# david-macmahon/BLDistributedDataProducts.jl

Hardware: AMD Instinct MI355X
Metric: filterbank GB/s reduced (node) + % HBM roofline, 8-bank 0000 band (higher is better)
Workload: dtype f32

## Files before the change

### bldistributeddataproducts.jl_amd/csrc/bslz4.hip

```cpp
#include <algorithm>
#include <cstring>
#include <vector>

#include "bldp_impl.h"

namespace {

inline uint32_t be32(const uint8_t *p) {
  return (uint32_t)p[0] << 24 | (uint32_t)p[1] << 16 | (uint32_t)p[2] << 8 | p[3];
}
inline uint64_t be64(const uint8_t *p) { return (uint64_t)be32(p) << 32 | be32(p + 4); }

__host__ __device__ inline uint64_t transpose8(uint64_t x) {
  uint64_t t;
  t = (x ^ (x >> 7)) & 0x00AA00AA00AA00AAull;
  x = x ^ t ^ (t << 7);
  t = (x ^ (x >> 14)) & 0x0000CCCC0000CCCCull;
  x = x ^ t ^ (t << 14);
  t = (x ^ (x >> 28)) & 0x00000000F0F0F0F0ull;
  x = x ^ t ^ (t << 28);
  return x;
}

int64_t lz4_block_host(const uint8_t *src, size_t slen, uint8_t *dst, size_t dcap) {
  size_t ip = 0, op = 0;
  while (ip < slen) {
    const uint8_t token = src[ip++];
    size_t lit = token >> 4;
    if (lit == 15) {
      uint8_t b;
      do {
        if (ip >= slen) return -1;
        b = src[ip++];
        lit += b;
      } while (b == 255);
    }
    if (ip + lit > slen || op + lit > dcap) return -1;
    memcpy(dst + op, src + ip, lit);
    ip += lit;
    op += lit;
    if (ip >= slen) break;
    if (ip + 2 > slen) return -1;
    const size_t off = (size_t)src[ip] | (size_t)src[ip + 1] << 8;
    ip += 2;
    size_t ml = token & 15;
    if (ml == 15) {
      uint8_t b;
      do {
        if (ip >= slen) return -1;
        b = src[ip++];
        ml += b;
      } while (b == 255);
    }
    ml += 4;
    if (off == 0 || off > op || op + ml > dcap) return -1;
    for (size_t i = 0; i < ml; ++i) dst[op + i] = dst[op - off + i];
    op += ml;
  }
  return (int64_t)op;
}

void bitunshuffle_host(const uint8_t *planes, uint8_t *out, size_t n, size_t es) {
  const size_t rowb = n / 8;
  for (size_t g = 0; g < rowb; ++g)
    for (size_t j = 0; j < es; ++j) {
      uint64_t x = 0;
      for (int k = 0; k < 8; ++k) x |= (uint64_t)planes[(j * 8 + k) * rowb + g] << (8 * k);
      x = transpose8(x);
      for (int t = 0; t < 8; ++t) out[(8 * g + t) * es + j] = (uint8_t)(x >> (8 * t));
    }
}

struct Task {
  uint64_t src;
  uint64_t dst;
  uint32_t clen;
  uint32_t nelem;
};
constexpr uint32_t RAW = 0xFFFFFFFFu;

struct ChunkDesc {
  uint64_t src, len, dst;
  uint64_t n, block;
  uint32_t nfull, last, tail;
  uint32_t task0;
};

int describe_chunk(const uint8_t *c, uint64_t len, uint64_t src, uint64_t dst, int es,
                   ChunkDesc *d) {
  if (len < 12) return bldp::set_error(BLDP_EINVAL, "bslz4: chunk shorter than its header");
  const uint64_t nb = be64(c);
  const uint32_t bb = be32(c + 8);
  if (nb % es || bb % es || bb == 0 || (bb / es) % 8 || bb > (1u << 24))
    return bldp::set_error(BLDP_EINVAL, "bslz4: bad header (bytes %llu, block %u, elem %d)",
                           (unsigned long long)nb, bb, es);
  d->src = src;
  d->len = len;
  d->dst = dst;
  d->n = nb / es;
  d->block = bb / es;
  d->nfull = (uint32_t)(d->n / d->block);
  uint64_t last = d->n % d->block;
  d->last = (uint32_t)(last - last % 8);
  d->tail = (uint32_t)(d->n - (uint64_t)d->nfull * d->block - d->last);
  return BLDP_OK;
}

inline uint32_t ntasks(const ChunkDesc &d) {
  return d.nfull + (d.last ? 1 : 0) + (d.tail ? 1 : 0);
}

__host__ __device__ inline uint32_t lz4_bound(uint32_t n) { return n + n / 255 + 16; }

__device__ inline uint32_t be32_dev(const uint8_t *p) {
  return (uint32_t)p[0] << 24 | (uint32_t)p[1] << 16 | (uint32_t)p[2] << 8 | p[3];
}

__global__ __launch_bounds__(64) void k_bslz4_plan(const uint8_t *__restrict__ comp,
                                                   const ChunkDesc *__restrict__ chunks,
                                                   int nchunk, int es, uint32_t cap,
                                                   Task *__restrict__ tasks, int *err) {
  const int k = blockIdx.x * 64 + threadIdx.x;
  if (k >= nchunk) return;
  const ChunkDesc d = chunks[k];
  uint64_t pos = d.src + 12, e = 0;
  const uint64_t end = d.src + d.len;
  const uint32_t nblk = d.nfull + (d.last ? 1 : 0);
  for (uint32_t b = 0; b < nblk; ++b) {
    const uint32_t ne = b < d.nfull ? (uint32_t)d.block : d.last;
    if (pos + 4 > end) { atomicOr(err, 2); return; }
    const uint32_t cl = be32_dev(comp + pos);
    if (cl > cap || pos + 4 + cl > end) { atomicOr(err, 2); return; }
    tasks[d.task0 + b] = Task{pos + 4, d.dst + e * es, cl, ne};
    pos += 4 + cl;
    e += ne;
  }
  if (pos + (uint64_t)d.tail * es != end) { atomicOr(err, 4); return; }
  if (d.tail) tasks[d.task0 + nblk] = Task{pos, d.dst + e * es, RAW, d.tail};
}

int plan_chunk(const uint8_t *c, uint64_t len, uint64_t src0, uint64_t dst0, int es,
               std::vector<Task> &tasks, uint64_t *out_bytes, uint32_t *max_block) {
  if (len < 12) return bldp::set_error(BLDP_EINVAL, "bslz4: chunk shorter than its header");
  const uint64_t nb = be64(c);
  const uint32_t bb = be32(c + 8);
  if (nb % es || bb % es || bb == 0 || (bb / es) % 8)
    return bldp::set_error(BLDP_EINVAL, "bslz4: bad header (bytes %llu, block %u, elem %d)",
                           (unsigned long long)nb, bb, es);
  const uint64_t n = nb / es, block = bb / es;
  uint64_t pos = 12, e = 0;
  const uint64_t nfull = n / block;
  uint64_t last = n % block;
  last -= last % 8;
  for (uint64_t k = 0; k < nfull + (last ? 1 : 0); ++k) {
    const uint64_t ne = k < nfull ? block : last;
    if (pos + 4 > len) return bldp::set_error(BLDP_EINVAL, "bslz4: truncated block header");
    const uint32_t cl = be32(c + pos);
    if (cl == RAW || pos + 4 + cl > len)
      return bldp::set_error(BLDP_EINVAL, "bslz4: block %llu overruns the chunk",
                             (unsigned long long)k);
    tasks.push_back(Task{src0 + pos + 4, dst0 + e * es, cl, (uint32_t)ne});
    *max_block = std::max<uint32_t>(*max_block, std::max<uint32_t>(cl, (uint32_t)(ne * es)));
    pos += 4 + cl;
    e += ne;
  }
  const uint64_t tail = n - e;
  if (pos + tail * es != len)
    return bldp::set_error(BLDP_EINVAL, "bslz4: %llu trailing bytes, expected %llu",
                           (unsigned long long)(len - pos), (unsigned long long)(tail * es));
  if (tail) tasks.push_back(Task{src0 + pos, dst0 + e * es, RAW, (uint32_t)tail});
  *out_bytes = nb;
  return BLDP_OK;
}

__global__ __launch_bounds__(64) void k_bslz4(const uint8_t *__restrict__ comp,
                                              const Task *__restrict__ tasks, int ntask,
                                              uint8_t *__restrict__ out, int es, uint32_t cap,
                                              int *err) {
  extern __shared__ uint8_t lds[];
  const int lane = threadIdx.x;
  if (*err & 6) return;
  const Task t = tasks[blockIdx.x];
  if (t.clen == RAW) {
    for (uint32_t i = lane; i < t.nelem * (uint32_t)es; i += 64) out[t.dst + i] = comp[t.src + i];
    return;
  }
  uint8_t *in = lds, *dec = lds + cap;
  const uint32_t clen = t.clen, nbytes = t.nelem * (uint32_t)es;
  if (clen > cap) {
    if (lane == 0) atomicOr(err, 1);
    return;
  }
  for (uint32_t i = lane; i < clen; i += 64) in[i] = comp[t.src + i];
  __syncthreads();
  uint32_t ip = 0, op = 0;
  bool bad = false;
  while (ip < clen) {
    const uint32_t token = in[ip++];
    uint32_t lit = token >> 4;
    if (lit == 15) {
      uint32_t b;
      do {
        if (ip >= clen) { bad = true; break; }
        b = in[ip++];
        lit += b;
      } while (b == 255);
      if (bad) break;
    }
    if (ip + lit > clen || op + lit > nbytes) { bad = true; break; }
    for (uint32_t i = lane; i < lit; i += 64) dec[op + i] = in[ip + i];
    ip += lit;
    op += lit;
    if (ip >= clen) break;
    if (ip + 2 > clen) { bad = true; break; }
    const uint32_t off = (uint32_t)in[ip] | (uint32_t)in[ip + 1] << 8;
    ip += 2;
    uint32_t ml = token & 15;
    if (ml == 15) {
      uint32_t b;
      do {
        if (ip >= clen) { bad = true; break; }
        b = in[ip++];
        ml += b;
      } while (b == 255);
      if (bad) break;
    }
    ml += 4;
    if (off == 0 || off > op || op + ml > nbytes) { bad = true; break; }
    __syncthreads();
    const uint32_t step = off < 64 ? off : 64;
    for (uint32_t r = 0; r < ml; r += step) {
      const uint32_t i = r + lane;
      if (lane < step && i < ml) dec[op + i] = dec[op - off + i];
      __syncthreads();
    }
    op += ml;
  }
  if (bad || op != nbytes) {
    if (lane == 0) atomicOr(err, 1);
    return;
  }
  __syncthreads();
  const uint32_t rowb = t.nelem / 8;
  if (es == 4) {
    for (uint32_t g = lane; g < rowb; g += 64) {
      uint32_t w[8] = {0, 0, 0, 0, 0, 0, 0, 0};
#pragma unroll
      for (int j = 0; j < 4; ++j) {
        uint64_t x = 0;
#pragma unroll
        for (int k = 0; k < 8; ++k) x |= (uint64_t)dec[(j * 8 + k) * rowb + g] << (8 * k);
        x = transpose8(x);
#pragma unroll
        for (int q = 0; q < 8; ++q) w[q] |= (uint32_t)((x >> (8 * q)) & 0xFF) << (8 * j);
      }
      uint32_t *o = reinterpret_cast<uint32_t *>(out + t.dst) + 8 * g;
#pragma unroll
      for (int q = 0; q < 8; ++q) o[q] = w[q];
    }
  } else {
    for (uint32_t g = lane; g < rowb; g += 64)
      for (int j = 0; j < es; ++j) {
        uint64_t x = 0;
        for (int k = 0; k < 8; ++k) x |= (uint64_t)dec[(j * 8 + k) * rowb + g] << (8 * k);
        x = transpose8(x);
        for (int q = 0; q < 8; ++q) out[t.dst + (8 * g + q) * es + j] = (uint8_t)(x >> (8 * q));
      }
  }
}

}

extern "C" {

BLDP_API int bldp_bslz4_info(const void *chunk, size_t nbytes, uint64_t *uncompressed_bytes,
                             uint32_t *block_bytes) {
  if (!chunk || nbytes < 12 || !uncompressed_bytes || !block_bytes)
    return bldp::set_error(BLDP_EINVAL, "bslz4: null pointer or short chunk");
  *uncompressed_bytes = be64((const uint8_t *)chunk);
  *block_bytes = be32((const uint8_t *)chunk + 8);
  return BLDP_OK;
}

BLDP_API int bldp_bslz4_decode_host(const void *chunk, size_t nbytes, int elem_size, void *out,
                                    size_t out_bytes) {
  if (!chunk || (!out && out_bytes) || elem_size <= 0)
    return bldp::set_error(BLDP_EINVAL, "bslz4: bad argument");
  std::vector<Task> tasks;
  uint64_t total = 0;
  uint32_t maxb = 0;
  int rc = plan_chunk((const uint8_t *)chunk, nbytes, 0, 0, elem_size, tasks, &total, &maxb);
  if (rc) return rc;
  if (total != out_bytes)
    return bldp::set_error(BLDP_EINVAL, "bslz4: chunk holds %llu bytes, output has %zu",
                           (unsigned long long)total, out_bytes);
  const uint8_t *c = (const uint8_t *)chunk;
  uint8_t *o = (uint8_t *)out;
  std::vector<uint8_t> dec(maxb);
  for (const Task &t : tasks) {
    const size_t nb = (size_t)t.nelem * elem_size;
    if (t.clen == RAW) {
      memcpy(o + t.dst, c + t.src, nb);
      continue;
    }
    if (lz4_block_host(c + t.src, t.clen, dec.data(), nb) != (int64_t)nb)
      return bldp::set_error(BLDP_EINVAL, "bslz4: corrupt LZ4 block at byte %llu",
                             (unsigned long long)t.src);
    bitunshuffle_host(dec.data(), o + t.dst, t.nelem, elem_size);
  }
  return BLDP_OK;
}

static int decode_launch(int nchunk, const uint8_t *comp_host, const uint8_t *comp_dev,
                         const uint64_t *chunk_off, const uint64_t *chunk_len, int elem_size,
                         uint8_t *out_dev, const uint64_t *out_off, const uint64_t *out_len,
                         int *derr_user, hipStream_t s, int **derr_used,
                         bldp::ScratchLease &lease, uint64_t host_base = 0) {
  if (nchunk < 0 || (nchunk && (!comp_host || !comp_dev || !chunk_off || !chunk_len ||
                                !out_dev || !out_off || !out_len)) ||
      elem_size <= 0 || elem_size > 64)
    return bldp::set_error(BLDP_EINVAL, "bslz4: bad argument");
  if (elem_size == 4 && ((uintptr_t)out_dev & 3))
    return bldp::set_error(BLDP_EINVAL, "bslz4: output must be 4-byte aligned");
  std::vector<ChunkDesc> descs(nchunk);
  uint64_t ntask = 0;
  uint32_t maxbb = 0;
  for (int k = 0; k < nchunk; ++k) {
    if (chunk_off[k] < host_base)
      return bldp::set_error(BLDP_EINVAL, "bslz4: chunk %d below the host staging base", k);
    int rc = describe_chunk(comp_host + (chunk_off[k] - host_base), chunk_len[k], chunk_off[k],
                            out_off[k],
                            elem_size, &descs[k]);
    if (rc) return rc;
    if (descs[k].n * (uint64_t)elem_size != out_len[k])
      return bldp::set_error(BLDP_EINVAL,
                             "bslz4: chunk %d decodes to %llu bytes, its output slot holds %llu",
                             k, (unsigned long long)(descs[k].n * elem_size),
                             (unsigned long long)out_len[k]);
    if (elem_size == 4 && (out_off[k] & 3))
      return bldp::set_error(BLDP_EINVAL, "bslz4: output offsets must be 4-byte aligned");
    descs[k].task0 = (uint32_t)ntask;
    ntask += ntasks(descs[k]);
    if (ntask > INT32_MAX) return bldp::set_error(BLDP_EINVAL, "bslz4: too many blocks");
    maxbb = std::max<uint32_t>(maxbb, (uint32_t)(descs[k].block * elem_size));
  }
  *derr_used = nullptr;
  if (ntask == 0) return BLDP_OK;
  const uint32_t cap = (lz4_bound(maxbb) + 15) & ~15u;
  if ((size_t)cap + (((size_t)maxbb + 15) & ~(size_t)15) > 64 * 1024)
    return bldp::set_error(BLDP_EINVAL, "bslz4: block of %u bytes exceeds the LDS plan", maxbb);
  const size_t dbytes = ((descs.size() * sizeof(ChunkDesc)) + 255) & ~(size_t)255;
  const size_t tbytes = ((ntask * sizeof(Task)) + 255) & ~(size_t)255;
  int rc = bldp::scratch_lease(s, dbytes + tbytes + 256, &lease);
  if (rc) return rc;
  void *ws = lease.ptr;
  ChunkDesc *ddesc = (ChunkDesc *)ws;
  Task *dtask = (Task *)((char *)ws + dbytes);
  int *derr = derr_user ? derr_user : (int *)((char *)ws + dbytes + tbytes);
  if (hipMemcpyAsync(ddesc, descs.data(), descs.size() * sizeof(ChunkDesc),
                     hipMemcpyHostToDevice, s) != hipSuccess ||
      (!derr_user && hipMemsetAsync(derr, 0, sizeof(int), s) != hipSuccess))
    return bldp::set_error(BLDP_EHIP, "bslz4: descriptor upload failed");
  hipLaunchKernelGGL(k_bslz4_plan, dim3((unsigned)((nchunk + 63) / 64)), dim3(64), 0, s,
                     comp_dev, ddesc, nchunk, elem_size, cap, dtask, derr);
  const uint32_t dcap = (maxbb + 15) & ~15u;
  hipLaunchKernelGGL(k_bslz4, dim3((unsigned)ntask), dim3(64), cap + dcap, s, comp_dev, dtask,
                     (int)ntask, out_dev, elem_size, cap, derr);
  hipError_t e = hipGetLastError();
  if (e != hipSuccess) return bldp::set_error(BLDP_EHIP, "bslz4 launch: %s", hipGetErrorString(e));
  *derr_used = derr;
  return BLDP_OK;
}

static int decode_error(int herr) {
  if (herr & 6) return bldp::set_error(BLDP_EINVAL, "bslz4: block table overruns a chunk");
  if (herr) return bldp::set_error(BLDP_EINVAL, "bslz4: corrupt LZ4 block on the device");
  return BLDP_OK;
}

BLDP_API int bldp_bslz4_decode_dev(int nchunk, const uint8_t *comp_host, const uint8_t *comp_dev,
                                   const uint64_t *chunk_off, const uint64_t *chunk_len,
                                   int elem_size, uint8_t *out_dev, const uint64_t *out_off,
                                   const uint64_t *out_len, void *stream) {
  hipStream_t s = (hipStream_t)stream;
  int *derr = nullptr;
  bldp::ScratchLease lease;
  int rc = decode_launch(nchunk, comp_host, comp_dev, chunk_off, chunk_len, elem_size, out_dev,
                         out_off, out_len, nullptr, s, &derr, lease);
  if (rc || !derr) return rc;
  int herr = 0;
  if (hipMemcpyAsync(&herr, derr, sizeof(int), hipMemcpyDeviceToHost, s) != hipSuccess ||
      hipStreamSynchronize(s) != hipSuccess)
    return bldp::set_error(BLDP_EHIP, "bslz4: synchronize failed");
  return decode_error(herr);
}

BLDP_API int bldp_bslz4_decode_dev_async(int nchunk, const uint8_t *comp_host,
                                         const uint8_t *comp_dev, const uint64_t *chunk_off,
                                         const uint64_t *chunk_len, int elem_size,
                                         uint8_t *out_dev, const uint64_t *out_off,
                                         const uint64_t *out_len, int *err_dev, void *stream) {
  if (!err_dev) return bldp::set_error(BLDP_EINVAL, "bslz4: null error word");
  int *derr = nullptr;
  bldp::ScratchLease lease;
  return decode_launch(nchunk, comp_host, comp_dev, chunk_off, chunk_len, elem_size, out_dev,
                       out_off, out_len, err_dev, (hipStream_t)stream, &derr, lease);
}

BLDP_API int bldp_bslz4_error(const int *err_dev, void *stream) {
  if (!err_dev) return bldp::set_error(BLDP_EINVAL, "bslz4: null error word");
  int herr = 0;
  hipStream_t s = (hipStream_t)stream;
  if (hipMemcpyAsync(&herr, err_dev, sizeof(int), hipMemcpyDeviceToHost, s) != hipSuccess ||
      hipStreamSynchronize(s) != hipSuccess)
    return bldp::set_error(BLDP_EHIP, "bslz4: synchronize failed");
  return decode_error(herr);
}

}

int bldp::bslz4_decode_async_at(int nchunk, const uint8_t *comp_host, uint64_t host_base,
                                const uint8_t *comp_dev, const uint64_t *chunk_off,
                                const uint64_t *chunk_len, int elem_size, uint8_t *out_dev,
                                const uint64_t *out_off, const uint64_t *out_len, int *err_dev,
                                hipStream_t s) {
  if (!err_dev) return bldp::set_error(BLDP_EINVAL, "bslz4: null error word");
  int *derr = nullptr;
  bldp::ScratchLease lease;
  return decode_launch(nchunk, comp_host, comp_dev, chunk_off, chunk_len, elem_size, out_dev,
                       out_off, out_len, err_dev, s, &derr, lease, host_base);
}
```

Before: 7394.

## Vectorize bslz4 staging, literal copies, match copies and bitshuffle output

Reworks the per-block LZ4 decode kernel in four places. Compressed input is staged into LDS with aligned 16-byte loads, literals are copied 8 bytes at a time, and match copies use a modular residue per lane so there is no per-step barrier. The es=4 bitshuffle transpose now reads dwords from LDS and writes 16-byte stores. These target byte-granular memory traffic and barrier stalls, at the cost of more registers (a 32-word array) and an extra 16 bytes of LDS per block.

```diff
diff --git a/bldistributeddataproducts.jl_amd/csrc/bslz4.hip b/bldistributeddataproducts.jl_amd/csrc/bslz4.hip
--- a/bldistributeddataproducts.jl_amd/csrc/bslz4.hip
+++ b/bldistributeddataproducts.jl_amd/csrc/bslz4.hip
@@ -3,6 +3,7 @@
 #include <vector>
 
 #include "bldp_impl.h"
+#include "bslz4_lanes.h"
 
 namespace {
 
@@ -173,25 +174,60 @@
   return BLDP_OK;
 }
 
+#ifndef BLDP_BSLZ4_STEPS
+#define BLDP_BSLZ4_STEPS 15
+#endif
+constexpr int kBslz4Steps = BLDP_BSLZ4_STEPS;
+
 __global__ __launch_bounds__(64) void k_bslz4(const uint8_t *__restrict__ comp,
                                               const Task *__restrict__ tasks, int ntask,
                                               uint8_t *__restrict__ out, int es, uint32_t cap,
                                               int *err) {
-  extern __shared__ uint8_t lds[];
-  const int lane = threadIdx.x;
+  extern __shared__ __attribute__((aligned(16))) uint8_t lds[];
+  constexpr int R = (int)kBslz4Rounds;
+  const uint32_t lane = threadIdx.x;
   if (*err & 6) return;
   const Task t = tasks[blockIdx.x];
   if (t.clen == RAW) {
     for (uint32_t i = lane; i < t.nelem * (uint32_t)es; i += 64) out[t.dst + i] = comp[t.src + i];
     return;
   }
-  uint8_t *in = lds, *dec = lds + cap;
   const uint32_t clen = t.clen, nbytes = t.nelem * (uint32_t)es;
   if (clen > cap) {
     if (lane == 0) atomicOr(err, 1);
     return;
   }
-  for (uint32_t i = lane; i < clen; i += 64) in[i] = comp[t.src + i];
+  const uint8_t *csrc = comp + t.src;
+  const uint32_t phase = (kBslz4Steps & 4) ? (uint32_t)((uintptr_t)csrc & 15) : 0u;
+  uint8_t *in = lds + phase, *dec = lds + cap + 16;
+  if (!(kBslz4Steps & 4)) {
+    for (uint32_t i = lane; i < clen; i += 64) in[i] = csrc[i];
+  } else {
+    const Bslz4Stage st = bslz4_stage_split(phase, clen);
+    uint8_t hb = 0;
+    uint32_t hk = 0;
+    if (clen) {
+      if (lane >= st.head && lane < st.head + st.tail) hk = st.body + lane;
+      else if (lane < st.head) hk = lane;
+      hb = csrc[hk];
+    }
+    const uint4 *g = reinterpret_cast<const uint4 *>(csrc + st.head);
+    uint4 *l = reinterpret_cast<uint4 *>(in + st.head);
+    const uint32_t nv = st.body >> 4;
+    for (uint32_t b = 0; b < nv; b += 64 * R) {
+      uint4 v[R];
+      uint32_t k[R];
+#pragma unroll
+      for (int u = 0; u < R; ++u) {
+        const uint32_t i = b + 64 * u + lane;
+        k[u] = i < nv ? i : nv - 1;
+        v[u] = g[k[u]];
+      }
+#pragma unroll
+      for (int u = 0; u < R; ++u) l[k[u]] = v[u];
+    }
+    if (clen) in[hk] = hb;
+  }
   __syncthreads();
   uint32_t ip = 0, op = 0;
   bool bad = false;
@@ -208,12 +244,23 @@
       if (bad) break;
     }
     if (ip + lit > clen || op + lit > nbytes) { bad = true; break; }
-    for (uint32_t i = lane; i < lit; i += 64) dec[op + i] = in[ip + i];
+    if (!(kBslz4Steps & 2)) {
+      for (uint32_t i = lane; i < lit; i += 64) dec[op + i] = in[ip + i];
+    } else {
+      const uint32_t n8 = lit >> 3;
+      for (uint32_t i = lane; i < n8; i += 64) {
+        uint64_t v;
+        __builtin_memcpy(&v, in + ip + 8 * i, 8);
+        __builtin_memcpy(dec + op + 8 * i, &v, 8);
+      }
+      if (lane < (lit & 7)) dec[op + 8 * n8 + lane] = in[ip + 8 * n8 + lane];
+    }
     ip += lit;
     op += lit;
     if (ip >= clen) break;
     if (ip + 2 > clen) { bad = true; break; }
-    const uint32_t off = (uint32_t)in[ip] | (uint32_t)in[ip + 1] << 8;
+    const uint32_t off = (uint32_t)__builtin_amdgcn_readfirstlane(
+        (int)((uint32_t)in[ip] | (uint32_t)in[ip + 1] << 8));
     ip += 2;
     uint32_t ml = token & 15;
     if (ml == 15) {
@@ -228,11 +275,29 @@
     ml += 4;
     if (off == 0 || off > op || op + ml > nbytes) { bad = true; break; }
     __syncthreads();
-    const uint32_t step = off < 64 ? off : 64;
-    for (uint32_t r = 0; r < ml; r += step) {
-      const uint32_t i = r + lane;
-      if (lane < step && i < ml) dec[op + i] = dec[op - off + i];
-      __syncthreads();
+    if (!(kBslz4Steps & 1)) {
+      const uint32_t step = off < 64 ? off : 64;
+      for (uint32_t r = 0; r < ml; r += step) {
+        const uint32_t i = r + lane;
+        if (lane < step && i < ml) dec[op + i] = dec[op - off + i];
+        __syncthreads();
+      }
+    } else {
+      const uint8_t *mb = dec + (op - off);
+      Bslz4Match m = bslz4_match_init(lane, off);
+      for (uint32_t b = 0; b < ml; b += 64 * R) {
+        uint8_t v[R];
+#pragma unroll
+        for (int u = 0; u < R; ++u) {
+          v[u] = mb[m.res];
+          m.res = bslz4_match_next(m.res, m.step, off);
+        }
+#pragma unroll
+        for (int u = 0; u < R; ++u) {
+          const uint32_t i = b + 64 * u + lane;
+          if (i < ml) dec[op + i] = v[u];
+        }
+      }
     }
     op += ml;
   }
@@ -242,7 +307,31 @@
   }
   __syncthreads();
   const uint32_t rowb = t.nelem / 8;
-  if (es == 4) {
+  if ((kBslz4Steps & 8) && bslz4_dword_path(es, rowb, (uint64_t)(uintptr_t)(out + t.dst))) {
+    const uint32_t nq = rowb >> 2;
+    for (uint32_t q = lane; q < nq; q += 64) {
+      uint32_t W[32];
+#pragma unroll
+      for (int p = 0; p < 32; ++p)
+        W[p] = *reinterpret_cast<const uint32_t *>(dec + (uint32_t)p * rowb + 4 * q);
+      uint4 *o = reinterpret_cast<uint4 *>(out + t.dst) + 8 * (size_t)q;
+#pragma unroll
+      for (int b = 0; b < 4; ++b) {
+        uint32_t w[8] = {0, 0, 0, 0, 0, 0, 0, 0};
+#pragma unroll
+        for (int j = 0; j < 4; ++j) {
+          uint64_t x = 0;
+#pragma unroll
+          for (int k = 0; k < 8; ++k) x |= (uint64_t)((W[j * 8 + k] >> (8 * b)) & 0xFF) << (8 * k);
+          x = transpose8(x);
+#pragma unroll
+          for (int e = 0; e < 8; ++e) w[e] |= (uint32_t)((x >> (8 * e)) & 0xFF) << (8 * j);
+        }
+        o[2 * b] = make_uint4(w[0], w[1], w[2], w[3]);
+        o[2 * b + 1] = make_uint4(w[4], w[5], w[6], w[7]);
+      }
+    }
+  } else if (es == 4) {
     for (uint32_t g = lane; g < rowb; g += 64) {
       uint32_t w[8] = {0, 0, 0, 0, 0, 0, 0, 0};
 #pragma unroll
@@ -347,7 +436,7 @@
   *derr_used = nullptr;
   if (ntask == 0) return BLDP_OK;
   const uint32_t cap = (lz4_bound(maxbb) + 15) & ~15u;
-  if ((size_t)cap + (((size_t)maxbb + 15) & ~(size_t)15) > 64 * 1024)
+  if ((size_t)cap + 16 + (((size_t)maxbb + 15) & ~(size_t)15) > 64 * 1024)
     return bldp::set_error(BLDP_EINVAL, "bslz4: block of %u bytes exceeds the LDS plan", maxbb);
   const size_t dbytes = ((descs.size() * sizeof(ChunkDesc)) + 255) & ~(size_t)255;
   const size_t tbytes = ((ntask * sizeof(Task)) + 255) & ~(size_t)255;
@@ -364,7 +453,7 @@
   hipLaunchKernelGGL(k_bslz4_plan, dim3((unsigned)((nchunk + 63) / 64)), dim3(64), 0, s,
                      comp_dev, ddesc, nchunk, elem_size, cap, dtask, derr);
   const uint32_t dcap = (maxbb + 15) & ~15u;
-  hipLaunchKernelGGL(k_bslz4, dim3((unsigned)ntask), dim3(64), cap + dcap, s, comp_dev, dtask,
+  hipLaunchKernelGGL(k_bslz4, dim3((unsigned)ntask), dim3(64), cap + 16 + dcap, s, comp_dev, dtask,
                      (int)ntask, out_dev, elem_size, cap, derr);
   hipError_t e = hipGetLastError();
   if (e != hipSuccess) return bldp::set_error(BLDP_EHIP, "bslz4 launch: %s", hipGetErrorString(e));
diff --git a/bldistributeddataproducts.jl_amd/csrc/bslz4_lanes.h b/bldistributeddataproducts.jl_amd/csrc/bslz4_lanes.h
--- /dev/null
+++ b/bldistributeddataproducts.jl_amd/csrc/bslz4_lanes.h
@@ -0,0 +1,55 @@
+#pragma once
+#include <cstdint>
+
+#if defined(__HIPCC__) || defined(__CUDACC__)
+#define BSLZ4_HD __host__ __device__
+#else
+#define BSLZ4_HD
+#endif
+
+constexpr uint32_t kBslz4Lanes = 64;
+constexpr uint32_t kBslz4Rounds = 4;
+
+
+struct Bslz4Match {
+  uint32_t res;
+  uint32_t step;
+};
+
+BSLZ4_HD inline Bslz4Match bslz4_match_init(uint32_t lane, uint32_t off) {
+  Bslz4Match s;
+  if (off >= kBslz4Lanes) {
+    s.res = lane;
+    s.step = off == kBslz4Lanes ? 0u : kBslz4Lanes;
+  } else {
+    const uint32_t m = 65536u / off + 1u;
+    s.res = lane - off * ((lane * m) >> 16);
+    s.step = kBslz4Lanes - off * ((kBslz4Lanes * m) >> 16);
+  }
+  return s;
+}
+
+BSLZ4_HD inline uint32_t bslz4_match_next(uint32_t res, uint32_t step, uint32_t off) {
+  res += step;
+  return res >= off ? res - off : res;
+}
+
+
+struct Bslz4Stage {
+  uint32_t head;
+  uint32_t body;
+  uint32_t tail;
+};
+
+BSLZ4_HD inline Bslz4Stage bslz4_stage_split(uint32_t phase, uint32_t clen) {
+  Bslz4Stage s;
+  const uint32_t h = (16u - (phase & 15u)) & 15u;
+  s.head = h < clen ? h : clen;
+  s.body = (clen - s.head) & ~15u;
+  s.tail = clen - s.head - s.body;
+  return s;
+}
+
+BSLZ4_HD inline bool bslz4_dword_path(int es, uint32_t rowb, uint64_t out_addr) {
+  return es == 4 && rowb != 0 && (rowb & 3u) == 0 && (out_addr & 15u) == 0;
+}
```

New measurement: 7385. Within noise of the previous version (-0.1%).
